# rti-team-imvia/RNb-NeuS-fork

Hardware: AMD Instinct MI355X
Metric: training rays/sec at 512 rays x 128 samples/ray (higher is better)
Workload: dtype f32; 1 GPU; DiLiGenT-MV-shaped synthetic rays, wmask_rnb.conf networks (8x256 SDF MLP + 2x256 albedo MLP), train_rnb step (render_rnb), 512 rays x (64+64) samples per GPU, 3 lights, geometric init, Adam; rays_per_gpu=512, global_rays=512, samples_per_ray=128, n_lights=3, no_albedo=False, parallelism=dp1, dp_loss=single process, deterministic=False, arithmetic=x2h, operand_bits=22, train_ops=rnb_loss_rnb + rnb_adam_step (one launch each)

## Files before the change

rnb-neus-fork_amd/csrc/color_h2.hip:

```cpp
#include "fused_common.hip.h"
#include "pe.hip.h"

namespace rnb {

struct ColH2Args {
  const float* pts;
  const float* nrm;
  long long M;
  const float* packed;
  const x3raw* w2;
  const H2Tab* h2tab;
  int id0;
  int F, pev, multires_view, Cinp, Co, squeeze;
  long long w_off[2], wT_off[2], b_off[2];
  long long wo_off, bo_off;
  int ldwo;
  float* cin;
  float* ac[2];
  unsigned* ac0_mask;
  float* alb;
  unsigned* smax;
  const float* albbar;
  float* zc[2];
  float* cinb;
  const float* x4;
  const float* nbar;
  float* geb;
  int multires, Ep;
  int keep_pe;
  unsigned* amax;
  float* dwo_part;
  float* dbo_part;
};

constexpr int CT = 64;

__device__ inline float relu_keep_nan(float x) { return x < 0.f ? 0.f : x; }

__device__ inline void col_mask_push(unsigned& m, float a) {
  asm("v_cmp_gt_f32 vcc, %1, 0\n\tv_addc_co_u32 %0, vcc, %0, %0, vcc" : "+v"(m) : "v"(a) : "vcc");
}
__device__ inline unsigned col_mask_bit(unsigned m, int ti, int r) { return (unsigned)(((int)(m << (ti * 16 + r))) >> 31); }

template <bool MASK>
__device__ inline float col_fwd_epilogue(const v16f (&acc)[2][2], float inv, const float* __restrict__ bias, float* X,
                                         float* __restrict__ out, int64_t row0, int n0, int lane, unsigned* __restrict__ mask_out) {
  const int h = lane >> 5, cl = lane & 31;
  const BufRsrc ro = tile_rsrc(out + (size_t)row0 * FH, CT * FH * 4);
  int amb = 0;
#pragma unroll
  for (int tj = 0; tj < 2; ++tj) {
    const int col = n0 + tj * 32 + cl;
    const float bc = bias[col];
    [[maybe_unused]] unsigned mk = 0u;
    const unsigned voff = (unsigned)(4 * h * FH + col) * 4u;
#pragma unroll
    for (int ti = 0; ti < 2; ++ti)
#pragma unroll
      for (int r = 0; r < 16; r += 2) {
        const int rowc = ti * 32 + (r & 3) + 8 * (r >> 2);
        const int row = rowc + 4 * h;
        const float a0 = relu_keep_nan(__builtin_fmaf(acc[ti][tj][r], inv, bc));
        const float a1 = relu_keep_nan(__builtin_fmaf(acc[ti][tj][r + 1], inv, bc));
        X[row * FP + col] = a0 * kH2ActScale;
        X[(row + 1) * FP + col] = a1 * kH2ActScale;
        h2_track2(amb, a0, a1);
        if constexpr (MASK) { col_mask_push(mk, a0); col_mask_push(mk, a1); }
        bstore(ro, voff, rowc * FH * 4, a0);
        bstore(ro, voff, (rowc + 1) * FH * 4, a1);
      }
    if constexpr (MASK) mask_out[tj] = mk;
  }
  return __builtin_bit_cast(float, amb);
}

__device__ inline void col_tile_rescale(int* flag, float am, float* wmx, float* X, int n0, int lane, int wave, unsigned* smax_slot,
                                        int tid, float& sa, float& isa) {
  sa = kH2ActScale;
  isa = 1.f / kH2ActScale;
  if (h2_flag_up(flag)) {
    am = wave_max(am);
    if (lane == 0) wmx[wave] = am;
    lds_barrier();
    const float tm = tile_max<4>(wmx);
    if (smax_slot != nullptr && tid == 0) amax_tile_commit(smax_slot, tm);
    if (tid == 0) *reinterpret_cast<volatile int*>(flag) = 0;
    x2h_dyn_scale(__builtin_bit_cast(unsigned, tm), sa, isa);
    const float f = sa * (1.f / kH2ActScale);
    for_each_acc<2, 2>(n0, lane, [&](int, int, int, int col, int, int row) { X[row * FP + col] *= f; });
    lds_barrier();
  }
}

__global__ __launch_bounds__(256, 2) void color_fwd_h2_kernel(ColH2Args g) {
  constexpr int NT = 256;
  __shared__ __attribute__((aligned(16))) float X[CT * FP];
  __shared__ float wmx[4];
  __shared__ int ovf[2];
  const int tid = threadIdx.x, lane = tid & 63;
  const int wave = wave_id();
  const int64_t row0 = (int64_t)blockIdx.x * CT;
  const int n0 = wave * 64;
  const int nks0 = g.Cinp >> 4, ksF = g.F >> 4;
  const x3raw* W0 = g.w2 + 2 * g.w_off[0];
  const x3raw* W1 = g.w2 + 2 * g.w_off[1];
  X3Mma<2, 2, 2> mm;
  const float iwsv = h2_iws_load(g.h2tab, lane);
  mm.request_at(W0, nks0, ksF, n0, lane);
  const int PW = g.Cinp - g.F;
  vf4 fr[CT * (FH / 4) / NT];
#pragma unroll
  for (int i = 0; i < CT * (FH / 4) / NT; ++i) {
    const int idx = tid + NT * i;
    fr[i] = *reinterpret_cast<const vf4*>(g.cin + (size_t)(row0 + (idx >> 6)) * g.Cinp + (idx & 63) * 4);
  }

  float pm;
  {
    const int p = tid & 63, part = tid >> 6, which = part >> 1, sub = part & 1;
    const int64_t row = row0 + p;
    float v[3] = {0.f, 0.f, 0.f};
    if (row < g.M) {
      if (which == 0) { v[0] = g.pts[row * 3]; v[1] = g.pts[row * 3 + 1]; v[2] = g.pts[row * 3 + 2]; }
      else { v[0] = g.nrm[row * 4]; v[1] = g.nrm[row * 4 + 1]; v[2] = g.nrm[row * 4 + 2]; }
    }
    float* xr = X + p * FP + which * g.pev;
    if (sub == 0) {
#pragma unroll
      for (int d = 0; d < 3; ++d) xr[d] = v[d] * kH2ActScale;
      if (which == 1)
        for (int c = 2 * g.pev; c < PW; ++c) X[p * FP + c] = 0.f;
    }
    pe_sincos(v, g.multires_view, sub, 2, [&](int c, float sn, float co) {
      xr[c] = sn * kH2ActScale;
      xr[c + 3] = co * kH2ActScale;
    });
    pm = fmaxf(fmaxf(fabsf(v[0]), fabsf(v[1])), fabsf(v[2]));
    const bool any = __builtin_amdgcn_ballot_w64(pm >= kH2ActLimit) != 0;
    if (lane == 0) wmx[wave] = any ? 1.f : 0.f;
    if (tid < 2) ovf[tid] = 0;
  }
  __syncthreads();
  float sa_p = kH2ActScale, isa_p = 1.f / kH2ActScale;
  if (tile_max<4>(wmx) != 0.f) {
    __syncthreads();
    pm = wave_max(pm);
    if (lane == 0) wmx[wave] = pm;
    __syncthreads();
    const float tm_p = fmaxf(tile_max<4>(wmx), 1.f);
    if (g.smax != nullptr && tid == 0) amax_tile_commit(g.smax + SMAX_CIN, tm_p);
    x2h_dyn_scale(__builtin_bit_cast(unsigned, tm_p), sa_p, isa_p);
    const float f = sa_p * (1.f / kH2ActScale);
    for (int idx = tid; idx < CT * PW; idx += NT) {
      const int r = idx / PW, c = idx - r * PW;
      X[r * FP + c] *= f;
    }
    __syncthreads();
  }
  for (int idx = tid; idx < CT * (PW / 4); idx += NT) {
    const int r = idx / (PW / 4), c4 = idx - r * (PW / 4);
    const vf4 v = *reinterpret_cast<const vf4*>(X + r * FP + c4 * 4) * isa_p;
    *reinterpret_cast<vf4*>(g.cin + (size_t)(row0 + r) * g.Cinp + g.F + c4 * 4) = v;
  }
  v16f acc[2][2];
  mm.run_at<false>(X, W0, nks0, ksF, PW >> 4, n0, lane, acc, W0, nks0, 0, n0);
  lds_barrier();
  float fm = 0.f;
#pragma unroll
  for (int i = 0; i < CT * (FH / 4) / NT; ++i) {
    const int idx = tid + NT * i;
    const vf4 v = fr[i];
    *reinterpret_cast<vf4*>(X + (idx >> 6) * FP + (idx & 63) * 4) = v * kH2ActScale;
    fm = fmaxf(fmaxf(fm, fmaxf(fabsf(v.x), fabsf(v.y))), fmaxf(fabsf(v.z), fabsf(v.w)));
  }
  h2_raise_flag(fm, &ovf[0], lane);
  __syncthreads();
  float sa = kH2ActScale, isa = 1.f / kH2ActScale;
  if (h2_flag_up(&ovf[0])) {
    fm = wave_max(fm);
    if (lane == 0) wmx[wave] = fm;
    __syncthreads();
    const float tm = tile_max<4>(wmx);
    if (g.smax != nullptr && tid == 0) amax_tile_commit(g.smax + SMAX_CIN, tm);
    if (tid == 0) ovf[0] = 0;
    x2h_dyn_scale(__builtin_bit_cast(unsigned, tm), sa, isa);
    const float f = sa * (1.f / kH2ActScale);
    for (int idx = tid; idx < CT * (FH / 4); idx += NT) {
      vf4* q = reinterpret_cast<vf4*>(X + (idx >> 6) * FP + (idx & 63) * 4);
      *q = *q * f;
    }
    __syncthreads();
  }
  if (sa != sa_p) {
    const float f = sa * isa_p;
#pragma unroll
    for (int ti = 0; ti < 2; ++ti)
#pragma unroll
      for (int tj = 0; tj < 2; ++tj) acc[ti][tj] = acc[ti][tj] * f;
  }
  mm.run_at<true>(X, W0, nks0, 0, ksF, n0, lane, acc, W1, FH >> 4, 0, n0);
  lds_barrier();
  {
    const float inv = isa * h2_iws_at(iwsv, g.id0);
    const float am = col_fwd_epilogue<true>(acc, inv, g.packed + g.b_off[0], X, g.ac[0], row0, n0, lane,
                                            g.ac0_mask + ((size_t)blockIdx.x * NT + tid) * 2);
    h2_raise_flag(am, &ovf[1], lane);
    lds_barrier();
    col_tile_rescale(&ovf[1], am, wmx, X, n0, lane, wave, g.smax ? g.smax + SMAX_AC : nullptr, tid, sa, isa);
  }
  mm.run(X, W1, FH, n0, lane, acc, nullptr, 0, 0);
  lds_barrier();
  {
    const float inv = isa * h2_iws_at(iwsv, g.id0 + 1);
    const float am = col_fwd_epilogue<false>(acc, inv, g.packed + g.b_off[1], X, g.ac[1], row0, n0, lane, nullptr);
    h2_raise_flag(am, &ovf[0], lane);
    lds_barrier();
    col_tile_rescale(&ovf[0], am, wmx, X, n0, lane, wave, g.smax ? g.smax + SMAX_AC + 1 : nullptr, tid, sa, isa);
  }
  {
    float w[4][4];
#pragma unroll
    for (int c = 0; c < 4; ++c)
#pragma unroll
      for (int u = 0; u < 4; ++u) w[c][u] = c < g.Co ? g.packed[g.wo_off + (long long)c * g.ldwo + lane + 64 * u] : 0.f;
    for (int rr = 0; rr < CT / 4; ++rr) {
      const int row = wave * (CT / 4) + rr;
      float sc[4] = {0.f, 0.f, 0.f, 0.f};
#pragma unroll
      for (int u = 0; u < 4; ++u) {
        const float a = X[row * FP + lane + 64 * u];
#pragma unroll
        for (int c = 0; c < 4; ++c) sc[c] = fmaf(a, w[c][u], sc[c]);
      }
#pragma unroll
      for (int c = 0; c < 4; ++c)
#pragma unroll
        for (int o = 32; o > 0; o >>= 1) sc[c] += __shfl_xor(sc[c], o, 64);
      if (lane < 4) {
        float v = 0.f;
        if (lane < g.Co) {
          const float s = lane == 0 ? sc[0] : lane == 1 ? sc[1] : lane == 2 ? sc[2] : sc[3];
          v = __builtin_fmaf(s, isa, g.packed[g.bo_off + lane]);
          if (g.squeeze) v = 1.f / (1.f + expf(-v));
        }
        g.alb[(row0 + row) * 4 + lane] = v;
      }
    }
  }
}

__global__ __launch_bounds__(256, 2) void color_bwd_h2_kernel(ColH2Args g) {
  __shared__ __attribute__((aligned(16))) float X[CT * FP];
  __shared__ __attribute__((aligned(16))) float ZO[CT * 4];
  __shared__ float wm[2][4];
  const int tid = threadIdx.x, lane = tid & 63;
  const int wave = wave_id();
  const int64_t row0 = (int64_t)blockIdx.x * CT;
  const int n0 = wave * 64;
  const long long left = g.M - row0;
  const int rows_ok = left >= CT ? CT : (int)(left < 0 ? 0 : left);
  const x3raw* W1T = g.w2 + 2 * g.wT_off[1];
  const x3raw* W0T = g.w2 + 2 * g.wT_off[0];
  const float iwsv = h2_iws_load(g.h2tab, lane);

  if (tid < CT) {
    const int64_t row = row0 + tid;
    const vf4 a4 = *reinterpret_cast<const vf4*>(g.alb + row * 4);
    const vf4 g4 = *reinterpret_cast<const vf4*>(g.albbar + row * 4);
    vf4 z;
#pragma unroll
    for (int c = 0; c < 4; ++c) z[c] = (c < g.Co && tid < rows_ok) ? g4[c] * (g.squeeze ? a4[c] * (1.f - a4[c]) : 1.f) : 0.f;
    *reinterpret_cast<vf4*>(ZO + tid * 4) = z;
  }
  AuxTile<2, 2> aA;
  prefetch_tile<2, 2>(g.ac[1], row0, n0, lane, aA);
  const vu2 mk0 = *reinterpret_cast<const vu2*>(g.ac0_mask + ((size_t)blockIdx.x * 256 + tid) * 2);
  __syncthreads();
  if (tid < g.Co) {
    float t = 0.f;
    for (int r = 0; r < CT; ++r) t += ZO[r * 4 + tid];
    g.dbo_part[(size_t)blockIdx.x * g.Co + tid] = t;
  }
  v16f acc[2][2];
  X3Mma<2, 2, 2> mm;
  {
    const int lane_a = opaque_lane(lane);
    const int h = lane_a >> 5, cl = lane_a & 31;
    const BufRsrc rz = tile_rsrc(g.zc[1] + (size_t)row0 * FH, CT * FH * 4);
    float ds[2][4], wo[2][4];
#pragma unroll
    for (int tj = 0; tj < 2; ++tj)
#pragma unroll
      for (int c = 0; c < 4; ++c) {
        wo[tj][c] = c < g.Co ? g.packed[g.wo_off + (long long)c * g.ldwo + n0 + tj * 32 + cl] : 0.f;
        ds[tj][c] = 0.f;
      }
#pragma unroll
    for (int ti = 0; ti < 2; ++ti)
#pragma unroll
      for (int r = 0; r < 16; ++r) {
        const int rowc = ti * 32 + (r & 3) + 8 * (r >> 2);
        const vf4 zo = *reinterpret_cast<const vf4*>(ZO + (rowc + 4 * h) * 4);
#pragma unroll
        for (int tj = 0; tj < 2; ++tj) {
          const int col = n0 + tj * 32 + cl;
          const float a = aA.v[ti][tj][r];
          const float t = fmaf(zo[0], wo[tj][0], fmaf(zo[1], wo[tj][1], fmaf(zo[2], wo[tj][2], zo[3] * wo[tj][3])));
          const float z = a > 0.f ? t : 0.f;
          acc[ti][tj][r] = z;
          bstore(rz, (unsigned)(4 * h * FH + col) * 4u, rowc * FH * 4, z);
#pragma unroll
          for (int c = 0; c < 4; ++c) ds[tj][c] = fmaf(zo[c], a, ds[tj][c]);
        }
      }
#pragma unroll
    for (int tj = 0; tj < 2; ++tj)
#pragma unroll
      for (int c = 0; c < 4; ++c) {
        const float tot = ds[tj][c] + __shfl_xor(ds[tj][c], 32, 64);
        if (lane < 32 && c < g.Co) g.dwo_part[((size_t)blockIdx.x * g.Co + c) * FH + n0 + tj * 32 + lane] = tot;
      }
    const float mr = wave_max(acc_absmax<2, 2>(acc, lane, rows_ok));
    if (lane == 0) wm[1][wave] = mr;
  }
  __syncthreads();
  float s, inv;
  {
    const float tmax = tile_scale<4>(wm[1], s, inv);
    if (tid == 0 && g.amax != nullptr) amax_tile_commit(g.amax + AMAX_ZC + 1, tmax);
  }
  for_each_acc<2, 2>(n0, lane, [&](int tj, int ti, int r, int col, int, int row) { X[row * FP + col] = acc[ti][tj][r] * s; });
  mm.request(W1T, FH, n0, lane);
  lds_barrier();
  mm.run(X, W1T, FH, n0, lane, acc, W0T, FH, n0);
  {
    const float unscale = inv * h2_iws_at(iwsv, g.id0 + 1);
    const int lane_e = opaque_lane(lane);
    const int h = lane_e >> 5;
    const BufRsrc rz = tile_rsrc(g.zc[0] + (size_t)row0 * FH, CT * FH * 4);
    for_each_acc<2, 2>(n0, lane_e, [&](int tj, int ti, int r, int col, int rowc, int) {
      const float z = __builtin_bit_cast(float, __builtin_bit_cast(unsigned, acc[ti][tj][r] * unscale) & col_mask_bit(mk0[tj], ti, r));
      bstore(rz, (unsigned)(4 * h * FH + col) * 4u, rowc * FH * 4, z);
      acc[ti][tj][r] = z;
    });
    const float mr = wave_max(acc_absmax<2, 2>(acc, lane_e, rows_ok));
    if (lane_e == 0) wm[0][wave] = mr;
  }
  lds_barrier();
  {
    const float tmax = tile_scale<4>(wm[0], s, inv);
    if (tid == 0 && g.amax != nullptr) amax_tile_commit(g.amax + AMAX_ZC, tmax);
  }
  for_each_acc<2, 2>(n0, lane, [&](int tj, int ti, int r, int col, int, int row) { X[row * FP + col] = acc[ti][tj][r] * s; });
  lds_barrier();
  const float unscale0 = inv * h2_iws_at(iwsv, g.id0);
  mm.run(X, W0T, FH, n0, lane, acc, nullptr, 0, 0);
  {
    const int lane_e = opaque_lane(lane);
    const int h = lane_e >> 5;
    const BufRsrc rc = tile_rsrc(g.cinb + (size_t)row0 * g.Cinp, CT * g.Cinp * 4);
    const unsigned rowb = (unsigned)g.Cinp * 4u;
    for_each_acc<2, 2>(n0, lane_e, [&](int tj, int ti, int r, int col, int rowc, int) {
      const float v = acc[ti][tj][r] * unscale0;
      bstore(rc, (unsigned)(4 * h) * rowb + (unsigned)col * 4u, rowc * rowb, v);
      acc[ti][tj][r] = v;
    });
    if (g.amax != nullptr) amax_commit(g.amax + AMAX_CINB, acc_absmax<2, 2>(acc, lane_e, rows_ok), lane_e);
  }
  v16f pacc[1][1];
  {
    X3Mma<1, 1, 2> mq;
    const int rt = wave & 1, ct = wave >> 1;
    mq.request(W0T, FH, g.F + 32 * ct, lane);
    mq.run(X + rt * 32 * FP, W0T, FH, g.F + 32 * ct, lane, pacc, nullptr, 0, 0);
  }
  lds_barrier();
  {
    const int rt = wave & 1, ct = wave >> 1, h = lane >> 5, cl = lane & 31;
#pragma unroll
    for (int r = 0; r < 16; ++r) X[(rt * 32 + (r & 3) + 8 * (r >> 2) + 4 * h) * FP + 32 * ct + cl] = pacc[0][0][r] * unscale0;
  }
  lds_barrier();
  if (g.keep_pe) {
    for (int idx = tid; idx < CT * 16; idx += 256) {
      const int r = idx >> 4, c4 = idx & 15;
      *reinterpret_cast<vf4*>(g.cinb + (size_t)(row0 + r) * g.Cinp + g.F + c4 * 4) = *reinterpret_cast<const vf4*>(X + r * FP + c4 * 4);
    }
  }
  if (g.geb == nullptr) return;
  {
    const int p = tid & 63, q = tid >> 6;
    const int64_t row = row0 + p;
    const bool ok = p < rows_ok;
    float* part = X + p * FP + 128;
    {
      const float* gq = X + p * FP + g.pev;
      float t[3] = {0.f, 0.f, 0.f};
      if (ok) pe_adjoint(g.nrm + row * 4, gq, g.multires_view, q, 4, t);
#pragma unroll
      for (int d = 0; d < 3; ++d) part[q * 3 + d] = t[d];
    }
    __syncthreads();
    float nb[3] = {0.f, 0.f, 0.f};
    if (ok) {
      const float* gq = X + p * FP + g.pev;
#pragma unroll
      for (int d = 0; d < 3; ++d) nb[d] = g.nbar[row * 4 + d] + gq[d] + ((part[d] + part[3 + d]) + (part[6 + d] + part[9 + d]));
    }
    float* o = X + p * FP + 64;
    if (q == 0) {
      o[0] = nb[0]; o[1] = nb[1]; o[2] = nb[2];
      for (int c = 3 + 6 * g.multires; c < g.Ep; ++c) o[c] = 0.f;
    }
    pe_tangent(g.x4 + row * 4, nb, g.multires, q, 4, [&](int c, float v0, float v1) {
      o[c] = v0;
      o[c + 3] = v1;
    });
  }
  __syncthreads();
  for (int idx = tid; idx < CT * (g.Ep / 4); idx += 256) {
    const int r = idx / (g.Ep / 4), c4 = idx - r * (g.Ep / 4);
    *reinterpret_cast<vf4*>(g.geb + (size_t)(row0 + r) * g.Ep + c4 * 4) = *reinterpret_cast<const vf4*>(X + r * FP + 64 + c4 * 4);
  }
}

bool color_h2_supported(const Layout& L) {
  return is_x2h(L) && !is_bf16(L) && L.F == FH && L.nc == 2 && L.Hc == FH && L.Hcp == FH && L.Cinp - L.F == 64 && L.Co >= 1 &&
         L.Co <= 4 && L.Ep == 64 && 2 * L.pev <= 64 && L.col[0].Kp == L.Cinp && L.col[1].Kp == FH;
}

static void col_fill(const Layout& L, const float* packed, PointBufs& pb, ColH2Args& g) {
  memset(&g, 0, sizeof(g));
  g.M = pb.M;
  g.packed = packed;
  g.w2 = x2h_mirror(L, packed);
  g.h2tab = h2_tab(L, packed);
  g.id0 = L.nh + 1;
  g.F = L.F;
  g.pev = L.pev;
  g.multires_view = L.multires_view;
  g.Cinp = L.Cinp;
  g.Co = L.Co;
  g.squeeze = L.squeeze;
  for (int l = 0; l < 2; ++l) {
    g.w_off[l] = L.col[l].w_off;
    g.wT_off[l] = L.col[l].wT_off;
    g.b_off[l] = L.col[l].b_off;
    g.ac[l] = pb.ac[l];
    g.zc[l] = pb.zc[l];
  }
  g.wo_off = L.colo.w_off;
  g.bo_off = L.colo.b_off;
  g.ldwo = L.colo.Kp;
  g.cin = pb.cin;
  g.alb = pb.alb;
  g.ac0_mask = pb.ac0_mask;
// ... 46 lines not shown
```

rnb-neus-fork_amd/csrc/fused.hip:

```cpp
#include <type_traits>

#include "fused_common.hip.h"
#include "pe.hip.h"

#ifndef RNB_X3_SCALAR_EPI
#define RNB_X3_SCALAR_EPI 0
#endif
#ifndef RNB_H2_SCALAR_EPI
#define RNB_H2_SCALAR_EPI 1
#endif
#ifndef RNB_H2_GUARD_AB
#define RNB_H2_GUARD_AB 0
#endif

namespace rnb {


template <int TI, bool SAVE, int NW = 4, bool X3 = false, bool H2 = false>
__global__ __launch_bounds__(64 * NW, NW == 8 ? 1 : 2) void fused_forward_kernel(FusedFwdArgs g) {
  static_assert(!H2 || X3, "x2h is a form of the split-operand path");
  constexpr float SA = H2 ? kH2ActScale : 1.f;
  constexpr int WP = H2 ? 2 : 3;
  constexpr int FT = 32 * TI;
  constexpr int NT = 64 * NW;
// ... 11 lines not shown
  const int n0 = wave * 32 * TJ;
  [[maybe_unused]] float sa = SA, isa = 1.f / SA;
  [[maybe_unused]] float iwsv = 0.f;
  if constexpr (H2) iwsv = h2_iws_load(g.h2tab, lane);

  [[maybe_unused]] float xm = 0.f;
  {
    constexpr int PARTS = NT / FT;
    const int p = tid % FT, part = tid / FT;
    const int64_t row = row0 + p;
    float x[3];
    sweep_point(g.grid, g.pts, row, g.M, g.net.scale, x);
    float* xr = X + p * FP;
    float* er = E + p * FEP;
    if (part == 0) {
      xr[0] = x[0] * SA; xr[1] = x[1] * SA; xr[2] = x[2] * SA;
      er[0] = x[0]; er[1] = x[1]; er[2] = x[2];
      for (int c = g.net.pe; c < g.net.Ep; ++c) xr[c] = 0.f;
      if (SAVE) {
        g.x4[row * 4] = x[0]; g.x4[row * 4 + 1] = x[1]; g.x4[row * 4 + 2] = x[2]; g.x4[row * 4 + 3] = 0.f;
      }
    }
    pe_sincos(x, g.net.multires, part, PARTS, [&](int c, float s, float co) {
      xr[c] = s * SA; xr[c + 3] = co * SA;
      er[c] = s; er[c + 3] = co;
    });
    if constexpr (H2) {
      xm = fmaxf(fmaxf(fabsf(x[0]), fabsf(x[1])), fabsf(x[2]));
      const bool any = __builtin_amdgcn_ballot_w64(xm >= kH2ActLimit) != 0;
      if (lane == 0) wmx[wave] = any ? 1.f : 0.f;
      if (tid < 2) ovf[tid] = 0;
    }
  }
  __syncthreads();
  if constexpr (H2) {
    if (tile_max<NW>(wmx) != 0.f) {
      __syncthreads();
      xm = wave_max(xm);
      if (lane == 0) wmx[wave] = xm;
      __syncthreads();
      const float tm = fmaxf(tile_max<NW>(wmx), 1.f);
      if (SAVE && g.smax != nullptr && tid == 0) amax_tile_commit(g.smax + SMAX_E, tm);
      x2h_dyn_scale(__builtin_bit_cast(unsigned, tm), sa, isa);
      const float f = sa * (1.f / SA);
      for (int idx = tid; idx < FT * g.net.Ep; idx += NT) {
        const int r = idx / g.net.Ep, c = idx - r * g.net.Ep;
        X[r * FP + c] *= f;
      }
      __syncthreads();
    }
  }
  if (SAVE) {
    for (int idx = tid; idx < FT * g.net.Ep; idx += NT) {
      const int r = idx / g.net.Ep, c = idx - r * g.net.Ep;
      g.e[(row0 + r) * g.net.Ep + c] = X[r * FP + c] * isa;
    }
  }

  const int h = lane >> 5, cl = lane & 31;
  v16f acc[TI][TJ];
  [[maybe_unused]] X3Mma<TI, TJ, WP> mm;
  if constexpr (X3) mm.request(g.w3 + WP * g.net.w_off[0], g.net.Kp[0], n0, lane);
  [[maybe_unused]] auto rescale_input = [&](float am_thread, int l_written) {
    am_thread = wave_max(am_thread);
    if (lane == 0) wmx[wave] = am_thread;
    lds_barrier();
    const float tm = tile_max<NW>(wmx);
    if (SAVE && g.smax != nullptr && tid == 0) amax_tile_commit(g.smax + SMAX_A + l_written, tm);
    if (tid == 0) ovf[l_written & 1] = 0;
    x2h_dyn_scale(__builtin_bit_cast(unsigned, tm), sa, isa);
    const float f = sa * (1.f / SA);
#pragma unroll
    for (int tj = 0; tj < TJ; ++tj)
#pragma unroll
      for (int ti = 0; ti < TI; ++ti)
#pragma unroll
        for (int r = 0; r < 16; ++r) X[(ti * 32 + (r & 3) + 8 * (r >> 2) + 4 * h) * FP + n0 + tj * 32 + cl] *= f;
    lds_barrier();
  };
  [[maybe_unused]] float am_prev = 0.f;
  for (int l = 0; l < g.net.nh; ++l) {
    [[maybe_unused]] int pend = 0;
    if constexpr (H2 && (RNB_H2_GUARD_AB == 0 || RNB_H2_GUARD_AB == 3)) {
      if (l > 0) pend = *reinterpret_cast<const volatile int*>(&ovf[(l - 1) & 1]);
    }
#if RNB_H2_GUARD_AB == 3
    [[maybe_unused]] float inv = H2 ? 1.f / (kH2ActScale * kH2WScale) : 1.f;
#else
    [[maybe_unused]] float inv = H2 ? isa * h2_iws_at(iwsv, l) : 1.f;
#endif
    if constexpr (X3) {
      const x3raw* wn = l + 1 < g.net.nh ? g.w3 + WP * g.net.w_off[l + 1] : (g.with_feat ? g.w3 + WP * g.net.wf_off : nullptr);
      mm.run(X, g.w3 + WP * g.net.w_off[l], g.net.Kp[l], n0, lane, acc, wn, FH, n0);
      if constexpr (H2 && (RNB_H2_GUARD_AB == 0 || RNB_H2_GUARD_AB == 3)) {
        if (__builtin_expect(__builtin_amdgcn_readfirstlane(pend) != 0, 0)) {
          lds_barrier();
          rescale_input(am_prev, l - 1);
#if RNB_H2_GUARD_AB != 3
          inv = isa * h2_iws_at(iwsv, l);
#endif
          mm.request(g.w3 + WP * g.net.w_off[l], g.net.Kp[l], n0, lane);
          mm.run(X, g.w3 + WP * g.net.w_off[l], g.net.Kp[l], n0, lane, acc, wn, FH, n0);
        }
      }
    } else layer_mma_nt<TI, NoHook, TJ>(X, g.packed + g.net.w_off[l], g.net.Kp[l], n0, lane, acc);
    if constexpr (NBUF == 1) lds_barrier();
    const float* bias = g.packed + g.net.b_off[l];
    const BufRsrc ra = tile_rsrc(SAVE ? g.a[l] + (size_t)row0 * FH : nullptr, FT * FH * 4);
    const BufRsrc rD = tile_rsrc(SAVE ? g.D[l] + (size_t)row0 * FH : nullptr, FT * FH * 4);
    const int n_real = g.net.n_real[l];
    const bool pe_tail = (l + 1 == g.net.skip);
    [[maybe_unused]] int amb = 0;
    [[maybe_unused]] float am = 0.f;
    auto column_tile = [&](auto full_c, int tj) {
      constexpr bool FULL = decltype(full_c)::value;
      const int col = n0 + tj * 32 + cl;
      const float bc = bias[col];
      const unsigned voff = (unsigned)(4 * h * FH + col) * 4u;
#pragma unroll
      for (int ti = 0; ti < TI; ++ti) {
#pragma unroll
        for (int r = 0; r < 16; r += 2) {
          const int rowc = ti * 32 + (r & 3) + 8 * (r >> 2);
          const int row = rowc + 4 * h;
          vf2 a, D;
          const vf2 z = H2 ? vf2{__builtin_fmaf(acc[ti][tj][r], inv, bc), __builtin_fmaf(acc[ti][tj][r + 1], inv, bc)}
                           : vf2{acc[ti][tj][r] + bc, acc[ti][tj][r + 1] + bc};
          constexpr bool SCALAR_EPI = H2 ? RNB_H2_SCALAR_EPI != 0 : (X3 && RNB_X3_SCALAR_EPI != 0);
          if constexpr (SAVE) softplus_aD_sel<SCALAR_EPI>(z, a, D);
          else a = softplus_a_sel<SCALAR_EPI>(z);
          if constexpr (!FULL) {
            if (col >= n_real) {
              const bool pe_col = pe_tail && col < n_real + g.net.pe;
              a = vf2{pe_col ? E[row * FEP + (col - n_real)] : 0.f, pe_col ? E[(row + 1) * FEP + (col - n_real)] : 0.f};
              D = vf2{0.f, 0.f};
              if constexpr (H2) am = fmaxf(am, fmaxf(fabsf(a.x), fabsf(a.y)));
            }
          }
          Y[row * FP + col] = a.x * SA;
          Y[(row + 1) * FP + col] = a.y * SA;
          if constexpr (H2 && RNB_H2_GUARD_AB != 1) h2_track2(amb, a.x, a.y);
          if (SAVE) {
            bstore(ra, voff, rowc * FH * 4, a.x);
            bstore(ra, voff, (rowc + 1) * FH * 4, a.y);
            bstore(rD, voff, rowc * FH * 4, D.x);
            bstore(rD, voff, (rowc + 1) * FH * 4, D.y);
          }
        }
      }
    };
#pragma unroll
    for (int tj = 0; tj < TJ; ++tj) {
      if (n0 + tj * 32 + 32 <= n_real) column_tile(std::true_type{}, tj);
      else column_tile(std::false_type{}, tj);
    }
    if constexpr (H2 && RNB_H2_GUARD_AB != 1) {
      am = fmaxf(am, __builtin_bit_cast(float, amb));
      h2_raise_flag(am, &ovf[l & 1], lane);
    }
    lds_barrier();
    if constexpr (H2) {
      sa = SA;
      isa = 1.f / SA;
      am_prev = am;
    }
    if constexpr (NBUF == 2) { float* t = X; X = Y; Y = t; }
  }
  if constexpr (H2 && RNB_H2_GUARD_AB == 0) {
    if (h2_flag_up(&ovf[(g.net.nh - 1) & 1])) rescale_input(am_prev, g.net.nh - 1);
  }

  {
    const float* ws = g.packed + g.net.wsdf_off;
    float w[4];
#pragma unroll
    for (int u = 0; u < 4; ++u) w[u] = ws[lane + 64 * u];
    const float bs = g.packed[g.net.bsdf_off];
    for (int rr = 0; rr < FT / NW; ++rr) {
      const int row = wave * (FT / NW) + rr;
      float s = 0.f;
#pragma unroll
      for (int u = 0; u < 4; ++u) s = fmaf(X[row * FP + lane + 64 * u], w[u], s);
#pragma unroll
      for (int o = 32; o > 0; o >>= 1) s += __shfl_xor(s, o, 64);
      if (lane == 0) {
        const float v = (H2 ? __builtin_fmaf(s, isa, bs) : s + bs) / g.net.scale;
        sweep_store_sdf(g.grid, g.sdf, row0, row, g.M, v);
      }
    }
  }
  if (g.with_feat) {
    [[maybe_unused]] const float inv = H2 ? isa * h2_iws_at(iwsv, g.net.nh) : 1.f;
    if constexpr (X3) mm.run(X, g.w3 + WP * g.net.wf_off, FH, n0, lane, acc, nullptr, 0, 0);
    else layer_mma_nt<TI, NoHook, TJ>(X, g.packed + g.net.wf_off, FH, n0, lane, acc);
    const float* bias = g.packed + g.net.bf_off;
    const BufRsrc rc = tile_rsrc(g.cin + (size_t)row0 * g.net.Cinp, FT * g.net.Cinp * 4);
    const unsigned rowb = (unsigned)g.net.Cinp * 4u;
#pragma unroll
    for (int tj = 0; tj < TJ; ++tj) {
      const int col = n0 + tj * 32 + cl;
      if (col < g.net.F) {
        const float bc = bias[col];
        const unsigned voff = (unsigned)(4 * h) * rowb + (unsigned)col * 4u;
#pragma unroll
        for (int ti = 0; ti < TI; ++ti) {
#pragma unroll
          for (int r = 0; r < 16; ++r) {
            const int rowc = ti * 32 + (r & 3) + 8 * (r >> 2);
            bstore(rc, voff, rowc * rowb, H2 ? __builtin_fmaf(acc[ti][tj][r], inv, bc) : acc[ti][tj][r] + bc);
          }
        }
      }
    }
  }
}

constexpr int kMaxX3 = 4 * RNB_MAX_LIN + 2;
struct X3Entry { long long off; int N, K, unit_begin, tperm, id, tr; };
struct X3Table { int n, total_units; X3Entry e[kMaxX3]; };
__global__ __launch_bounds__(256) void x3_pack_kernel(const float* __restrict__ src, X3Table t, x3raw* __restrict__ dst,
                                                      H2Tab* __restrict__ tab) {
  __shared__ float wmx[4];
  const int u = blockIdx.x * 256 + threadIdx.x;
  const bool live = u < t.total_units;
  int ei = 0;
  while (ei + 1 < t.n && u >= t.e[ei + 1].unit_begin) ++ei;
  const X3Entry en = t.e[ei];
  float m = 0.f;
  if (live) {
    const int lu = u - en.unit_begin;
    const int frag = lu >> 6, lane = lu & 63;
    const int nks = en.K >> 4;
    const int nt = frag / nks, ks = frag - nt * nks;
    const int c = lane & 31, h = lane >> 5;
    const float* sp = src + en.off + (size_t)(nt * 32 + c) * en.K + ks * 16 + h * (en.tperm ? 4 : 8);
    const vf4 x0 = *reinterpret_cast<const vf4*>(sp), x1 = *reinterpret_cast<const vf4*>(sp + (en.tperm ? 8 : 4));
    vu4x hi, mid, lo;
    x3_split8(x0, x1, hi, mid, lo);
    x3raw* dp = dst + 3 * en.off + ((size_t)frag * 3 * 64 + lane) * 8;
    *reinterpret_cast<vu4x*>(dp) = hi;
    *reinterpret_cast<vu4x*>(dp + 512) = mid;
    *reinterpret_cast<vu4x*>(dp + 1024) = lo;
    m = fmaxf(fmaxf(fmaxf(fabsf(x0.x), fabsf(x0.y)), fmaxf(fabsf(x0.z), fabsf(x0.w))),
              fmaxf(fmaxf(fabsf(x1.x), fabsf(x1.y)), fmaxf(fabsf(x1.z), fabsf(x1.w))));
  }
  if (tab == nullptr) return;
  const bool rec = live && en.id >= 0 && !en.tr;
  const int blk0 = blockIdx.x * 256;
  const bool whole = en.unit_begin <= blk0 && blk0 + 256 <= en.unit_begin + en.N * en.K / 8;
#pragma unroll
  for (int o = 32; o > 0; o >>= 1) m = fmaxf(m, __shfl_xor(m, o, 64));
  if (!whole) {
    if (rec && (threadIdx.x & 63) == 0) amax_tile_commit(tab->wmax + en.id, m);
    return;
  }
  if ((threadIdx.x & 63) == 0) wmx[threadIdx.x >> 6] = m;
  __syncthreads();
  if (rec && threadIdx.x == 0) amax_tile_commit(tab->wmax + en.id, fmaxf(fmaxf(wmx[0], wmx[1]), fmaxf(wmx[2], wmx[3])));
}
__device__ inline float x2h_weight_scale(unsigned mbits, float& inv) {
  float s = kH2WScale;
  inv = 1.f / kH2WScale;
  const int ef = (int)(mbits >> 23);
  if (ef >= 127 + 6 && ef < 255) x2h_dyn_scale(mbits, s, inv);
  return s;
}
__global__ void x2h_pack_kernel(const float* __restrict__ src, X3Table t, x3raw* __restrict__ dst, H2Tab* __restrict__ tab) {
  const int u = blockIdx.x * blockDim.x + threadIdx.x;
  if (u >= t.total_units) return;
  int ei = 0;
  while (ei + 1 < t.n && u >= t.e[ei + 1].unit_begin) ++ei;
  const X3Entry en = t.e[ei];
  const int lu = u - en.unit_begin;
  const int frag = lu >> 6, lane = lu & 63;
  const int nks = en.K >> 4;
  const int nt = frag / nks, ks = frag - nt * nks;
  const int c = lane & 31, h = lane >> 5;
  float inv;
  const float sw = x2h_weight_scale(tab->wmax[en.id], inv);
  if (lu == 0 && !en.tr) { tab->ws[en.id] = sw; tab->iws[en.id] = inv; }
  const float* sp = src + en.off + (size_t)(nt * 32 + c) * en.K + ks * 16 + h * (en.tperm ? 4 : 8);
  vu4x hi, lo;
  x2h_split8(*reinterpret_cast<const vf4*>(sp) * sw, *reinterpret_cast<const vf4*>(sp + (en.tperm ? 8 : 4)) * sw, hi, lo);
  x3raw* dp = dst + 2 * en.off + ((size_t)frag * 2 * 64 + lane) * 8;
  *reinterpret_cast<vu4x*>(dp) = hi;
// ... 93 lines not shown
```

rnb-neus-fork_amd/csrc/fused_common.hip.h:

```cpp
#pragma once
#include <stdlib.h>

#include "gemm.hip.h"
#include "rnb_internal.h"

namespace rnb {

constexpr int FH = 256;
constexpr int FP = FH + 4;
constexpr int FEP = 40;

struct FusedFwdArgs {
  const float* pts;
  int64_t M;
  const float* packed;
  const x3raw* w3;
  SdfNetArgs net;
  int with_feat;
  float* cin;
  float* sdf;
  float* x4;
  float* e;
  float* a[RNB_MAX_LIN];
  float* D[RNB_MAX_LIN];
  GridGen grid;
  const H2Tab* h2tab;
  unsigned* smax;
};

constexpr float kH2ActLimit = 256.f;
__device__ inline float wave_max(float m) {
#pragma unroll
  for (int o = 32; o > 0; o >>= 1) m = fmaxf(m, __shfl_xor(m, o, 64));
  return m;
}
template <int NW>
__device__ inline float tile_max(const float* wm) {
  float m = wm[0];
#pragma unroll
  for (int w = 1; w < NW; ++w) m = fmaxf(m, wm[w]);
  return m;
}
template <int NW>
__device__ inline float tile_scale(const float* wm, float& s, float& inv_s) {
  const float m = tile_max<NW>(wm);
  x2h_dyn_scale(__builtin_bit_cast(unsigned, m), s, inv_s);
  return m;
}
__device__ inline void h2_track2(int& m, float a, float b) {
  asm("v_max3_i32 %0, %1, %2, %3" : "=v"(m) : "v"(m), "v"(a), "v"(b));
}
__device__ inline void h2_raise_flag(float mine, int* flag, int lane) {
  if (__builtin_amdgcn_ballot_w64(mine >= kH2ActLimit) != 0 && lane == 0) *reinterpret_cast<volatile int*>(flag) = 1;
}
__device__ inline bool h2_flag_up(const int* flag) {
  return __builtin_expect(__builtin_amdgcn_readfirstlane(*reinterpret_cast<const volatile int*>(flag)) != 0, 0);
}
__device__ inline float h2_iws_load(const H2Tab* tab, int lane) { return tab->iws[lane < kH2TabSlots ? lane : 0]; }
__device__ inline float h2_iws_at(float iwsv, int id) {
  return __builtin_bit_cast(float, __builtin_amdgcn_readlane(__builtin_bit_cast(int, iwsv), id));
}
__device__ inline void amax_tile_commit(unsigned* slot, float m) {
  (void)__hip_atomic_fetch_max(slot, __builtin_bit_cast(unsigned, m), __ATOMIC_RELAXED, __HIP_MEMORY_SCOPE_AGENT);
}

template <int TJ>
__device__ inline void load_b_block(const float* __restrict__ W, int K, int n0, int Q, int lane, vf4 (&b)[TJ][4]) {
  const int j = lane & 31, h = lane >> 5;
#pragma unroll
  for (int tj = 0; tj < TJ; ++tj) {
    const float* p = W + (size_t)(n0 + tj * 32 + j) * K + Q * 32 + h * 16;
#pragma unroll
    for (int q = 0; q < 4; ++q) b[tj][q] = *reinterpret_cast<const vf4*>(p + q * 4);
  }
}

__device__ inline int opaque_lane(int v) { asm volatile("" : "+v"(v)); return v; }

struct NoHook {
  __device__ void operator()() const {}
};

template <int TI, bool FIRST = false, int TJ = 2>
__device__ inline void mma_block(const float* __restrict__ X, int Q, int i, int h, const vf4 (&b)[TJ][4],
                                 v16f (&acc)[TI][TJ]) {
#pragma unroll
  for (int q = 0; q < 4; ++q) {
    vf4 a[TI];
#pragma unroll
    for (int ti = 0; ti < TI; ++ti)
      a[ti] = *reinterpret_cast<const vf4*>(X + (ti * 32 + i) * FP + Q * 32 + h * 16 + q * 4);
#pragma unroll
    for (int c = 0; c < 4; ++c) {
#pragma unroll
      for (int tj = 0; tj < TJ; ++tj)
#pragma unroll
        for (int ti = 0; ti < TI; ++ti) {
          if (FIRST && q == 0 && c == 0) {
            const v16f zero = {0.f, 0.f, 0.f, 0.f, 0.f, 0.f, 0.f, 0.f, 0.f, 0.f, 0.f, 0.f, 0.f, 0.f, 0.f, 0.f};
            acc[ti][tj] = __builtin_amdgcn_mfma_f32_32x32x2f32(a[ti][c], b[tj][q][c], zero, 0, 0, 0);
          } else {
            acc[ti][tj] = __builtin_amdgcn_mfma_f32_32x32x2f32(a[ti][c], b[tj][q][c], acc[ti][tj], 0, 0, 0);
          }
        }
    }
    __builtin_amdgcn_sched_barrier(0);
  }
}

template <int TI, class Hook = NoHook, int TJ = 2>
__device__ inline void layer_mma_nt(const float* __restrict__ X, const float* __restrict__ W, int K, int n0, int lane,
                                    v16f (&acc)[TI][TJ], Hook hook = Hook(), int hook_late = 0) {
  const int i = lane & 31, h = lane >> 5;
  const int nQ = K / 32;
  const int hookQ = hook_late ? (nQ >= 2 ? nQ - 2 : 0) : (nQ > 2 ? 1 : 0);
  vf4 b0[TJ][4], b1[TJ][4];
  load_b_block<TJ>(W, K, n0, 0, lane, b0);
  load_b_block<TJ>(W, K, n0, 1, lane, b1);
  if (hookQ == 0) hook();
  mma_block<TI, true, TJ>(X, 0, i, h, b0, acc);
  if (2 < nQ) load_b_block<TJ>(W, K, n0, 2, lane, b0);
  if (hookQ == 1) hook();
  mma_block<TI, false, TJ>(X, 1, i, h, b1, acc);
  for (int Q = 2; Q < nQ; Q += 2) {
    load_b_block<TJ>(W, K, n0, Q + 1, lane, b1);
    if (Q == hookQ) hook();
    mma_block<TI, false, TJ>(X, Q, i, h, b0, acc);
    if (Q + 2 < nQ) load_b_block<TJ>(W, K, n0, Q + 2, lane, b0);
    if (Q + 1 == hookQ) hook();
    mma_block<TI, false, TJ>(X, Q + 1, i, h, b1, acc);
  }
}

template <int TI, bool FIRST>
__device__ inline void ring_block(const float* __restrict__ X, const float* __restrict__ p0,
                                  const float* __restrict__ p1, int Q, int Qn, int i, int h, vf4 (&b)[2][4],
                                  v16f (&acc)[TI][2]) {
#pragma unroll
  for (int q = 0; q < 4; ++q) {
// ... 240 lines not shown
```

Measured before the change: 200,800 rays/s.

## Hoist bias and weight loads ahead of MMAs and relax LDS overflow flags

```diff
diff --git a/rnb-neus-fork_amd/csrc/color_h2.hip b/rnb-neus-fork_amd/csrc/color_h2.hip
--- a/rnb-neus-fork_amd/csrc/color_h2.hip
+++ b/rnb-neus-fork_amd/csrc/color_h2.hip
@@ -1,3 +1,5 @@
+#include <type_traits>
+
 #include "fused_common.hip.h"
 #include "pe.hip.h"
 
@@ -37,13 +39,17 @@
 
 __device__ inline float relu_keep_nan(float x) { return x < 0.f ? 0.f : x; }
 
+__device__ inline void col_bias_request(const float* __restrict__ bias, int n0, int lane, float (&bc)[2]) {
+#pragma unroll
+  for (int tj = 0; tj < 2; ++tj) bc[tj] = bias[n0 + tj * 32 + (lane & 31)];
+}
 __device__ inline void col_mask_push(unsigned& m, float a) {
   asm("v_cmp_gt_f32 vcc, %1, 0\n\tv_addc_co_u32 %0, vcc, %0, %0, vcc" : "+v"(m) : "v"(a) : "vcc");
 }
 __device__ inline unsigned col_mask_bit(unsigned m, int ti, int r) { return (unsigned)(((int)(m << (ti * 16 + r))) >> 31); }
 
 template <bool MASK>
-__device__ inline float col_fwd_epilogue(const v16f (&acc)[2][2], float inv, const float* __restrict__ bias, float* X,
+__device__ inline float col_fwd_epilogue(const v16f (&acc)[2][2], float inv, const float (&bias)[2], float* X,
                                          float* __restrict__ out, int64_t row0, int n0, int lane, unsigned* __restrict__ mask_out) {
   const int h = lane >> 5, cl = lane & 31;
   const BufRsrc ro = tile_rsrc(out + (size_t)row0 * FH, CT * FH * 4);
@@ -51,7 +57,7 @@
 #pragma unroll
   for (int tj = 0; tj < 2; ++tj) {
     const int col = n0 + tj * 32 + cl;
-    const float bc = bias[col];
+    const float bc = bias[tj];
     [[maybe_unused]] unsigned mk = 0u;
     const unsigned voff = (unsigned)(4 * h * FH + col) * 4u;
 #pragma unroll
@@ -74,6 +80,16 @@
   return __builtin_bit_cast(float, amb);
 }
 
+template <int T>
+__device__ inline void prefetch_rows32(const BufRsrc rs, int n0, int lane, float (&v)[2][16]) {
+  const int h = lane >> 5, cl = lane & 31;
+#pragma unroll
+  for (int tj = 0; tj < 2; ++tj)
+#pragma unroll
+    for (int r = 0; r < 16; ++r)
+      v[tj][r] = bload(rs, (unsigned)(4 * h * FH + n0 + tj * 32 + cl) * 4u, (T * 32 + (r & 3) + 8 * (r >> 2)) * FH * 4);
+}
+
 __device__ inline void col_tile_rescale(int* flag, float am, float* wmx, float* X, int n0, int lane, int wave, unsigned* smax_slot,
                                         int tid, float& sa, float& isa) {
   sa = kH2ActScale;
@@ -84,7 +100,7 @@
     lds_barrier();
     const float tm = tile_max<4>(wmx);
     if (smax_slot != nullptr && tid == 0) amax_tile_commit(smax_slot, tm);
-    if (tid == 0) *reinterpret_cast<volatile int*>(flag) = 0;
+    if (tid == 0) h2_flag_write(flag, 0);
     x2h_dyn_scale(__builtin_bit_cast(unsigned, tm), sa, isa);
     const float f = sa * (1.f / kH2ActScale);
     for_each_acc<2, 2>(n0, lane, [&](int, int, int, int col, int, int row) { X[row * FP + col] *= f; });
@@ -198,31 +214,38 @@
 #pragma unroll
       for (int tj = 0; tj < 2; ++tj) acc[ti][tj] = acc[ti][tj] * f;
   }
+  float bc[2];
+  col_bias_request(g.packed + g.b_off[0], n0, lane, bc);
   mm.run_at<true>(X, W0, nks0, 0, ksF, n0, lane, acc, W1, FH >> 4, 0, n0);
   lds_barrier();
   {
     const float inv = isa * h2_iws_at(iwsv, g.id0);
-    const float am = col_fwd_epilogue<true>(acc, inv, g.packed + g.b_off[0], X, g.ac[0], row0, n0, lane,
+    const float am = col_fwd_epilogue<true>(acc, inv, bc, X, g.ac[0], row0, n0, lane,
                                             g.ac0_mask + ((size_t)blockIdx.x * NT + tid) * 2);
     h2_raise_flag(am, &ovf[1], lane);
     lds_barrier();
     col_tile_rescale(&ovf[1], am, wmx, X, n0, lane, wave, g.smax ? g.smax + SMAX_AC : nullptr, tid, sa, isa);
   }
+  col_bias_request(g.packed + g.b_off[1], n0, lane, bc);
   mm.run(X, W1, FH, n0, lane, acc, nullptr, 0, 0);
   lds_barrier();
+  float w[4][4];
+#pragma unroll
+  for (int c = 0; c < 4; ++c)
+#pragma unroll
+    for (int u = 0; u < 4; ++u) {
+      const float t = g.packed[g.wo_off + (long long)min(c, g.Co - 1) * g.ldwo + lane + 64 * u];
+      w[c][u] = c < g.Co ? t : 0.f;
+    }
+  const float bo = g.packed[g.bo_off + min(lane, g.Co - 1)];
   {
     const float inv = isa * h2_iws_at(iwsv, g.id0 + 1);
-    const float am = col_fwd_epilogue<false>(acc, inv, g.packed + g.b_off[1], X, g.ac[1], row0, n0, lane, nullptr);
+    const float am = col_fwd_epilogue<false>(acc, inv, bc, X, g.ac[1], row0, n0, lane, nullptr);
     h2_raise_flag(am, &ovf[0], lane);
     lds_barrier();
     col_tile_rescale(&ovf[0], am, wmx, X, n0, lane, wave, g.smax ? g.smax + SMAX_AC + 1 : nullptr, tid, sa, isa);
   }
   {
-    float w[4][4];
-#pragma unroll
-    for (int c = 0; c < 4; ++c)
-#pragma unroll
-      for (int u = 0; u < 4; ++u) w[c][u] = c < g.Co ? g.packed[g.wo_off + (long long)c * g.ldwo + lane + 64 * u] : 0.f;
     for (int rr = 0; rr < CT / 4; ++rr) {
       const int row = wave * (CT / 4) + rr;
       float sc[4] = {0.f, 0.f, 0.f, 0.f};
@@ -240,7 +263,7 @@
         float v = 0.f;
         if (lane < g.Co) {
           const float s = lane == 0 ? sc[0] : lane == 1 ? sc[1] : lane == 2 ? sc[2] : sc[3];
-          v = __builtin_fmaf(s, isa, g.packed[g.bo_off + lane]);
+          v = __builtin_fmaf(s, isa, bo);
           if (g.squeeze) v = 1.f / (1.f + expf(-v));
         }
         g.alb[(row0 + row) * 4 + lane] = v;
@@ -272,9 +295,18 @@
     for (int c = 0; c < 4; ++c) z[c] = (c < g.Co && tid < rows_ok) ? g4[c] * (g.squeeze ? a4[c] * (1.f - a4[c]) : 1.f) : 0.f;
     *reinterpret_cast<vf4*>(ZO + tid * 4) = z;
   }
-  AuxTile<2, 2> aA;
-  prefetch_tile<2, 2>(g.ac[1], row0, n0, lane, aA);
+  const BufRsrc ra1 = tile_rsrc(g.ac[1] + (size_t)row0 * FH, CT * FH * 4);
+  float aA0[2][16], aA1[2][16];
+  prefetch_rows32<0>(ra1, n0, lane, aA0);
   const vu2 mk0 = *reinterpret_cast<const vu2*>(g.ac0_mask + ((size_t)blockIdx.x * 256 + tid) * 2);
+  float wo[2][4];
+#pragma unroll
+  for (int tj = 0; tj < 2; ++tj)
+#pragma unroll
+    for (int c = 0; c < 4; ++c) {
+      const float w = g.packed[g.wo_off + (long long)min(c, g.Co - 1) * g.ldwo + n0 + tj * 32 + (lane & 31)];
+      wo[tj][c] = c < g.Co ? w : 0.f;
+    }
   __syncthreads();
   if (tid < g.Co) {
     float t = 0.f;
@@ -283,20 +315,20 @@
   }
   v16f acc[2][2];
   X3Mma<2, 2, 2> mm;
+  prefetch_rows32<1>(ra1, n0, lane, aA1);
+  mm.request(W1T, FH, n0, lane);
+  __builtin_amdgcn_sched_barrier(0);
   {
     const int lane_a = opaque_lane(lane);
     const int h = lane_a >> 5, cl = lane_a & 31;
     const BufRsrc rz = tile_rsrc(g.zc[1] + (size_t)row0 * FH, CT * FH * 4);
-    float ds[2][4], wo[2][4];
+    float ds[2][4];
 #pragma unroll
     for (int tj = 0; tj < 2; ++tj)
 #pragma unroll
-      for (int c = 0; c < 4; ++c) {
-        wo[tj][c] = c < g.Co ? g.packed[g.wo_off + (long long)c * g.ldwo + n0 + tj * 32 + cl] : 0.f;
-        ds[tj][c] = 0.f;
-      }
-#pragma unroll
-    for (int ti = 0; ti < 2; ++ti)
+      for (int c = 0; c < 4; ++c) ds[tj][c] = 0.f;
+    auto rows32 = [&](auto ti_c, const float (&a32)[2][16]) {
+      constexpr int ti = decltype(ti_c)::value;
 #pragma unroll
       for (int r = 0; r < 16; ++r) {
         const int rowc = ti * 32 + (r & 3) + 8 * (r >> 2);
@@ -304,7 +336,7 @@
 #pragma unroll
         for (int tj = 0; tj < 2; ++tj) {
           const int col = n0 + tj * 32 + cl;
-          const float a = aA.v[ti][tj][r];
+          const float a = a32[tj][r];
           const float t = fmaf(zo[0], wo[tj][0], fmaf(zo[1], wo[tj][1], fmaf(zo[2], wo[tj][2], zo[3] * wo[tj][3])));
           const float z = a > 0.f ? t : 0.f;
           acc[ti][tj][r] = z;
@@ -312,7 +344,17 @@
 #pragma unroll
           for (int c = 0; c < 4; ++c) ds[tj][c] = fmaf(zo[c], a, ds[tj][c]);
         }
+        if ((r & 3) == 3) {
+#pragma unroll
+          for (int tj = 0; tj < 2; ++tj)
+#pragma unroll
+            for (int c = 0; c < 4; ++c) asm volatile("" : "+v"(ds[tj][c]));
+          __builtin_amdgcn_sched_barrier(0);
+        }
       }
+    };
+    rows32(std::integral_constant<int, 0>{}, aA0);
+    rows32(std::integral_constant<int, 1>{}, aA1);
 #pragma unroll
     for (int tj = 0; tj < 2; ++tj)
 #pragma unroll
@@ -330,7 +372,6 @@
     if (tid == 0 && g.amax != nullptr) amax_tile_commit(g.amax + AMAX_ZC + 1, tmax);
   }
   for_each_acc<2, 2>(n0, lane, [&](int tj, int ti, int r, int col, int, int row) { X[row * FP + col] = acc[ti][tj][r] * s; });
-  mm.request(W1T, FH, n0, lane);
   lds_barrier();
   mm.run(X, W1T, FH, n0, lane, acc, W0T, FH, n0);
   {
@@ -354,6 +395,8 @@
   for_each_acc<2, 2>(n0, lane, [&](int tj, int ti, int r, int col, int, int row) { X[row * FP + col] = acc[ti][tj][r] * s; });
   lds_barrier();
   const float unscale0 = inv * h2_iws_at(iwsv, g.id0);
+  X3Mma<1, 1, 2> mq;
+  mq.request(W0T, FH, g.F + 32 * (wave >> 1), lane);
   mm.run(X, W0T, FH, n0, lane, acc, nullptr, 0, 0);
   {
     const int lane_e = opaque_lane(lane);
@@ -369,9 +412,7 @@
   }
   v16f pacc[1][1];
   {
-    X3Mma<1, 1, 2> mq;
     const int rt = wave & 1, ct = wave >> 1;
-    mq.request(W0T, FH, g.F + 32 * ct, lane);
     mq.run(X + rt * 32 * FP, W0T, FH, g.F + 32 * ct, lane, pacc, nullptr, 0, 0);
   }
   lds_barrier();
diff --git a/rnb-neus-fork_amd/csrc/fused.hip b/rnb-neus-fork_amd/csrc/fused.hip
--- a/rnb-neus-fork_amd/csrc/fused.hip
+++ b/rnb-neus-fork_amd/csrc/fused.hip
@@ -117,13 +117,20 @@
   for (int l = 0; l < g.net.nh; ++l) {
     [[maybe_unused]] int pend = 0;
     if constexpr (H2 && (RNB_H2_GUARD_AB == 0 || RNB_H2_GUARD_AB == 3)) {
-      if (l > 0) pend = *reinterpret_cast<const volatile int*>(&ovf[(l - 1) & 1]);
+      if (l > 0) pend = h2_flag_read(&ovf[(l - 1) & 1]);
     }
 #if RNB_H2_GUARD_AB == 3
     [[maybe_unused]] float inv = H2 ? 1.f / (kH2ActScale * kH2WScale) : 1.f;
 #else
     [[maybe_unused]] float inv = H2 ? isa * h2_iws_at(iwsv, l) : 1.f;
 #endif
+    const float* bias = g.packed + g.net.b_off[l];
+    float bcv[TJ];
+#pragma unroll
+    for (int tj = 0; tj < TJ; ++tj) bcv[tj] = bias[n0 + tj * 32 + cl];
+    const BufRsrc ra = tile_rsrc(SAVE ? g.a[l] + (size_t)row0 * FH : nullptr, FT * FH * 4);
+    const BufRsrc rD = tile_rsrc(SAVE ? g.D[l] + (size_t)row0 * FH : nullptr, FT * FH * 4);
+    const int n_real = g.net.n_real[l];
     if constexpr (X3) {
       const x3raw* wn = l + 1 < g.net.nh ? g.w3 + WP * g.net.w_off[l + 1] : (g.with_feat ? g.w3 + WP * g.net.wf_off : nullptr);
       mm.run(X, g.w3 + WP * g.net.w_off[l], g.net.Kp[l], n0, lane, acc, wn, FH, n0);
@@ -140,17 +147,13 @@
       }
     } else layer_mma_nt<TI, NoHook, TJ>(X, g.packed + g.net.w_off[l], g.net.Kp[l], n0, lane, acc);
     if constexpr (NBUF == 1) lds_barrier();
-    const float* bias = g.packed + g.net.b_off[l];
-    const BufRsrc ra = tile_rsrc(SAVE ? g.a[l] + (size_t)row0 * FH : nullptr, FT * FH * 4);
-    const BufRsrc rD = tile_rsrc(SAVE ? g.D[l] + (size_t)row0 * FH : nullptr, FT * FH * 4);
-    const int n_real = g.net.n_real[l];
     const bool pe_tail = (l + 1 == g.net.skip);
     [[maybe_unused]] int amb = 0;
     [[maybe_unused]] float am = 0.f;
     auto column_tile = [&](auto full_c, int tj) {
       constexpr bool FULL = decltype(full_c)::value;
       const int col = n0 + tj * 32 + cl;
-      const float bc = bias[col];
+      const float bc = bcv[tj];
       const unsigned voff = (unsigned)(4 * h * FH + col) * 4u;
 #pragma unroll
       for (int ti = 0; ti < TI; ++ti) {
@@ -211,6 +214,7 @@
 #pragma unroll
     for (int u = 0; u < 4; ++u) w[u] = ws[lane + 64 * u];
     const float bs = g.packed[g.net.bsdf_off];
+    float mine = 0.f;
     for (int rr = 0; rr < FT / NW; ++rr) {
       const int row = wave * (FT / NW) + rr;
       float s = 0.f;
@@ -218,24 +222,28 @@
       for (int u = 0; u < 4; ++u) s = fmaf(X[row * FP + lane + 64 * u], w[u], s);
 #pragma unroll
       for (int o = 32; o > 0; o >>= 1) s += __shfl_xor(s, o, 64);
-      if (lane == 0) {
-        const float v = (H2 ? __builtin_fmaf(s, isa, bs) : s + bs) / g.net.scale;
-        sweep_store_sdf(g.grid, g.sdf, row0, row, g.M, v);
-      }
+      if (lane == rr) mine = s;
+    }
+    if (lane < FT / NW) {
+      const float v = (H2 ? __builtin_fmaf(mine, isa, bs) : mine + bs) / g.net.scale;
+      sweep_store_sdf(g.grid, g.sdf, row0, wave * (FT / NW) + lane, g.M, v);
     }
   }
   if (g.with_feat) {
     [[maybe_unused]] const float inv = H2 ? isa * h2_iws_at(iwsv, g.net.nh) : 1.f;
+    const float* bias = g.packed + g.net.bf_off;
+    float bcv[TJ];
+#pragma unroll
+    for (int tj = 0; tj < TJ; ++tj) bcv[tj] = n0 + tj * 32 + cl < g.net.F ? bias[n0 + tj * 32 + cl] : 0.f;
     if constexpr (X3) mm.run(X, g.w3 + WP * g.net.wf_off, FH, n0, lane, acc, nullptr, 0, 0);
     else layer_mma_nt<TI, NoHook, TJ>(X, g.packed + g.net.wf_off, FH, n0, lane, acc);
-    const float* bias = g.packed + g.net.bf_off;
     const BufRsrc rc = tile_rsrc(g.cin + (size_t)row0 * g.net.Cinp, FT * g.net.Cinp * 4);
     const unsigned rowb = (unsigned)g.net.Cinp * 4u;
 #pragma unroll
     for (int tj = 0; tj < TJ; ++tj) {
       const int col = n0 + tj * 32 + cl;
       if (col < g.net.F) {
-        const float bc = bias[col];
+        const float bc = bcv[tj];
         const unsigned voff = (unsigned)(4 * h) * rowb + (unsigned)col * 4u;
 #pragma unroll
         for (int ti = 0; ti < TI; ++ti) {
diff --git a/rnb-neus-fork_amd/csrc/fused_common.hip.h b/rnb-neus-fork_amd/csrc/fused_common.hip.h
--- a/rnb-neus-fork_amd/csrc/fused_common.hip.h
+++ b/rnb-neus-fork_amd/csrc/fused_common.hip.h
@@ -50,11 +50,18 @@
 __device__ inline void h2_track2(int& m, float a, float b) {
   asm("v_max3_i32 %0, %1, %2, %3" : "=v"(m) : "v"(m), "v"(a), "v"(b));
 }
+typedef __attribute__((address_space(3))) int lds_int;
+__device__ inline int h2_flag_read(const int* flag) {
+  return __hip_atomic_load((const lds_int*)flag, __ATOMIC_RELAXED, __HIP_MEMORY_SCOPE_WORKGROUP);
+}
+__device__ inline void h2_flag_write(int* flag, int v) {
+  __hip_atomic_store((lds_int*)flag, v, __ATOMIC_RELAXED, __HIP_MEMORY_SCOPE_WORKGROUP);
+}
 __device__ inline void h2_raise_flag(float mine, int* flag, int lane) {
-  if (__builtin_amdgcn_ballot_w64(mine >= kH2ActLimit) != 0 && lane == 0) *reinterpret_cast<volatile int*>(flag) = 1;
+  if (__builtin_amdgcn_ballot_w64(mine >= kH2ActLimit) != 0 && lane == 0) h2_flag_write(flag, 1);
 }
 __device__ inline bool h2_flag_up(const int* flag) {
-  return __builtin_expect(__builtin_amdgcn_readfirstlane(*reinterpret_cast<const volatile int*>(flag)) != 0, 0);
+  return __builtin_expect(__builtin_amdgcn_readfirstlane(h2_flag_read(flag)) != 0, 0);
 }
 __device__ inline float h2_iws_load(const H2Tab* tab, int lane) { return tab->iws[lane < kH2TabSlots ? lane : 0]; }
 __device__ inline float h2_iws_at(float iwsv, int id) {
```

Measured after the change: 203,200 rays/s, median of 6. 1.2% higher.
